# Leonhard111/M3L

Measured on AMD Instinct MI355X. Metric: MAE fwd+bwd samples/sec (image+tactile), higher is better.
Workload: dtype bf16; 1 GPU; BASELINE configs[1]: VTT vision+tactile MAE, 64x64 RGB + 2x32x32 tactile, ViT-Tiny 192/12/3/768 + decoder 192/4/3/768, mask 0.75; batch_per_gpu=256, global_batch=256, parallelism=dp1, grad_allreduce=none (one rank), rccl_ranks=0, step=zero_grad + mask + fwd + bwd + grad all-reduce + Adam

## Files before the change

### __graft_entry__.py

```python
import os
import subprocess
import sys

ROOT = os.path.dirname(os.path.abspath(__file__))
CSRC = os.path.join(ROOT, "m3l_amd", "csrc")
LIB = os.path.join(ROOT, "m3l_amd", "lib", "libm3l_amd.so")
SOURCES = ["gemm.hip", "wgrad.hip", "gemm_rowln.hip", "attention.hip", "attn_block.hip", "mlp_block.hip", "enc_mega.hip", "t192.hip", "conv.hip", "elementwise.hip", "mae_plan.hip", "mae_step.hip", "prof.hip", "err.hip", "comm.hip"]


OBJ = os.path.join(ROOT, "build", "obj")
HIPCC_FLAGS = ["--offload-arch=gfx950", "-O3", "-std=c++17", "-fPIC", "-Wno-unused-value", "-fno-slp-vectorize"]


def _headers():
    return [os.path.join(CSRC, f) for f in os.listdir(CSRC) if f.endswith((".h", ".cuh"))] + [os.path.join(ROOT, "include", "m3l_amd.h")]


def _compile_stale(force: bool):
    os.makedirs(OBJ, exist_ok=True)
    flags_file = os.path.join(OBJ, "flags.txt")
    flags = " ".join(HIPCC_FLAGS)
    if not os.path.exists(flags_file) or open(flags_file).read() != flags:
        force = True
        open(flags_file, "w").write(flags)
    hdr_t = max(os.path.getmtime(h) for h in _headers())
    jobs = []
    for src in SOURCES:
        obj = os.path.join(OBJ, src.replace(".hip", ".o"))
        s = os.path.join(CSRC, src)
        if force or not os.path.exists(obj) or os.path.getmtime(obj) < max(os.path.getmtime(s), hdr_t):
            jobs.append((src, ["hipcc"] + HIPCC_FLAGS + ["-c", s, "-o", obj]))
    running, failed = [], []
    while jobs or running:
        while jobs and len(running) < 8:
            src, cmd = jobs.pop(0)
            running.append((src, subprocess.Popen(cmd, cwd=CSRC, stdout=subprocess.PIPE, stderr=subprocess.STDOUT, text=True)))
        src, pr = running.pop(0)
        out, _ = pr.communicate()
        if pr.returncode != 0:
            failed.append(src)
# ... 88 lines not shown
```

### include/m3l_amd.h

```cpp
#ifndef M3L_AMD_H
#define M3L_AMD_H
#include <stddef.h>
#include <stdint.h>

#ifdef __cplusplus
extern "C" {
#endif

#define M3L_MAX_TACTILES 8

typedef struct m3l_geom {
    int image_h, image_w, image_patch, image_channels;
    int tactile_h, tactile_w, tactile_patch, tactile_channels;
    int num_tactiles;
    int use_vision;
    int use_tactile;
} m3l_geom;

typedef struct m3l_tf_cfg {
    int dim, depth, heads, mlp_dim;
    int project_out;
    int dtype;
    int dim_head;
} m3l_tf_cfg;

typedef struct m3l_dropout {
    float p;
    uint64_t seed;
} m3l_dropout;

int m3l_version(void);
int m3l_last_error(char* buf, size_t n);
int m3l_set_rowln(int enable);
int m3l_set_attn_block(int mode);
int m3l_set_enc_mega(int mode);
void m3l_set_attn_phase_buffer(void* dev_buf);
int m3l_set_defer_join(int on);
int m3l_set_wgrad_inline(int on);
int m3l_side_join(void* stream);
int m3l_comm_available(void);
int m3l_comm_unique_id(void* out128);
int m3l_comm_init(const void* id128, int rank, int world);
int m3l_comm_world(void);
int m3l_comm_allreduce(float* buf, size_t count, void* after_stream);
int m3l_comm_destroy(void);
int m3l_side_fork(void* after_stream, void** side_out);
int m3l_side_mark_pending(void);
void* m3l_side_stream(void);
int m3l_side_pending(void);
int m3l_set_drop_h(int on);
int m3l_set_t192(int on);
int m3l_set_t192_tt(int tt);
int m3l_set_residual_bf16(int on);
int m3l_set_t192_stagger(int lead_mask, int prio_mask);

int m3l_mask_counts(const m3l_geom* g, double ratio, int* counts_host);
int m3l_mask_sample(const m3l_geom* g, double ratio, int B, const float* const* noise, int64_t* masked, int64_t* unmasked,
                    void* stream);

int m3l_mask_sample_counts(const m3l_geom* g, int nm_img, int nm_tac, int B, const float* const* noise, int64_t* masked,
                           int64_t* unmasked, void* stream);

size_t m3l_embed_ws_bytes(const m3l_geom* g, int D, int dtype, int B, int L);
int m3l_embed_fwd(const m3l_geom* g, int D, int dtype, int B, int L, int cnt_img, const int64_t* idx, const float* image,
                  const float* const* tactiles, const void* const* tensors, void* ws, float* tokens, void* stream);
int m3l_embed_bwd(const m3l_geom* g, int D, int dtype, int B, int L, int cnt_img, const int64_t* idx, const float* image,
                  const float* const* tactiles, const void* const* tensors, void* ws, const float* dtokens, float* const* grads,
                  void* stream);

size_t m3l_transformer_ws_bytes(const m3l_tf_cfg* c, int B, int n);
int m3l_transformer_fwd(const m3l_tf_cfg* c, int B, int n, const float* x_in, const void* const* tensors, void* ws, void* y_t,
// ... 155 lines not shown
```

### m3l_amd/_lib.py

```python
import ctypes as C
import os

_HERE = os.path.dirname(os.path.abspath(__file__))
LIB_PATH = os.environ.get("M3L_LIB_PATH") or os.path.join(_HERE, "lib", "libm3l_amd.so")

c_p = C.c_void_p
c_i = C.c_int
c_sz = C.c_size_t


class Geom(C.Structure):
    _fields_ = [(n, c_i) for n in ("image_h", "image_w", "image_patch", "image_channels", "tactile_h", "tactile_w",
                                   "tactile_patch", "tactile_channels", "num_tactiles", "use_vision", "use_tactile")]


class CnnCfg(C.Structure):
    _fields_ = [(n, c_i) for n in ("in_channels", "height", "width", "dim", "tactile", "dtype")]


class TfCfg(C.Structure):
    _fields_ = [(n, c_i) for n in ("dim", "depth", "heads", "mlp_dim", "project_out", "dtype", "dim_head")]


class MaeCfg(C.Structure):
    _fields_ = [("geom", Geom), ("enc", TfCfg), ("dec", TfCfg), ("masking_ratio", C.c_double), ("early_conv", c_i), ("learned_pos", c_i)]


class Dropout(C.Structure):
    _fields_ = [("p", C.c_float), ("seed", C.c_uint64)]


class CommPlan(C.Structure):
    _fields_ = [("flat", c_p), ("total", C.c_long), ("min_bucket", C.c_long), ("layers_per_chunk", c_i), ("n_stages", c_i),
                ("stage_end", C.POINTER(C.c_long)), ("sent_out", C.POINTER(C.c_long))]


_SIGS = {
    "m3l_version": (c_i, []),
    "m3l_last_error": (c_i, [C.c_char_p, c_sz]),
    "m3l_set_rowln": (c_i, [c_i]),
    "m3l_set_attn_block": (c_i, [c_i]),
    "m3l_set_attn_phase_buffer": (None, [c_p]),
    "m3l_set_enc_mega": (c_i, [c_i]),
    "m3l_set_drop_h": (c_i, [c_i]),
    "m3l_set_direct_conv": (c_i, [c_i]),
    "m3l_set_t192": (c_i, [c_i]),
    "m3l_set_t192_tt": (c_i, [c_i]),
    "m3l_set_t192_stagger": (c_i, [c_i, c_i]),
    "m3l_set_residual_bf16": (c_i, [c_i]),
    "m3l_set_defer_join": (c_i, [c_i]),
    "m3l_set_wgrad_inline": (c_i, [c_i]),
    "m3l_side_join": (c_i, [c_p]),
    "m3l_side_stream": (c_p, []),
    "m3l_side_fork": (c_i, [c_p, C.POINTER(c_p)]),
    "m3l_side_mark_pending": (c_i, []),
    "m3l_comm_available": (c_i, []),
    "m3l_comm_unique_id": (c_i, [c_p]),
    "m3l_comm_init": (c_i, [c_p, c_i, c_i]),
    "m3l_comm_world": (c_i, []),
    "m3l_comm_allreduce": (c_i, [c_p, c_sz, c_p]),
    "m3l_comm_destroy": (c_i, []),
    "m3l_side_pending": (c_i, []),
    "m3l_mask_counts": (c_i, [C.POINTER(Geom), C.c_double, C.POINTER(c_i)]),
    "m3l_mask_sample": (c_i, [C.POINTER(Geom), C.c_double, c_i, c_p, c_p, c_p, c_p]),
    "m3l_mask_sample_counts": (c_i, [C.POINTER(Geom), c_i, c_i, c_i, c_p, c_p, c_p, c_p]),
    "m3l_embed_ws_bytes": (c_sz, [C.POINTER(Geom), c_i, c_i, c_i, c_i]),
    "m3l_embed_fwd": (c_i, [C.POINTER(Geom), c_i, c_i, c_i, c_i, c_i, c_p, c_p, c_p, c_p, c_p, c_p, c_p]),
    "m3l_embed_bwd": (c_i, [C.POINTER(Geom), c_i, c_i, c_i, c_i, c_i, c_p, c_p, c_p, c_p, c_p, c_p, c_p, c_p]),
    "m3l_transformer_ws_bytes": (c_sz, [C.POINTER(TfCfg), c_i, c_i]),
    "m3l_transformer_fwd": (c_i, [C.POINTER(TfCfg), c_i, c_i, c_p, c_p, c_p, c_p, c_p, c_p]),
    "m3l_transformer_bwd": (c_i, [C.POINTER(TfCfg), c_i, c_i, c_p, c_p, c_p, c_p, c_i, c_p, c_p, c_p]),
    "m3l_transformer_bwd_range": (c_i, [C.POINTER(TfCfg), c_i, c_i, c_p, c_p, c_p, c_p, c_i, c_p, c_p, c_i, c_i, c_p]),
    "m3l_transformer_ws_bytes_dropout": (c_sz, [C.POINTER(TfCfg), c_i, c_i, C.POINTER(Dropout)]),
    "m3l_transformer_fwd_dropout": (c_i, [C.POINTER(TfCfg), c_i, c_i, c_p, c_p, c_p, c_p, c_p, C.POINTER(Dropout), c_p]),
    "m3l_transformer_bwd_dropout": (c_i, [C.POINTER(TfCfg), c_i, c_i, c_p, c_p, c_p, c_p, c_i, c_p, c_p, C.POINTER(Dropout), c_p]),
    "m3l_transformer_bwd_range_dropout": (c_i, [C.POINTER(TfCfg), c_i, c_i, c_p, c_p, c_p, c_p, c_i, c_p, c_p, c_i, c_i, C.POINTER(Dropout), c_p]),
    "m3l_frozen_vit_ws_bytes": (c_sz, [C.POINTER(TfCfg), c_i, c_i]),
    "m3l_frozen_vit_fwd": (c_i, [C.POINTER(TfCfg), C.c_float, c_i, c_i, c_p, c_p, c_p, c_p, c_p]),
    "m3l_unshuffle_ws_bytes": (c_sz, [C.POINTER(Geom), c_i, c_i, c_i, c_i, c_i, c_i]),
    "m3l_unshuffle_fwd": (c_i, [C.POINTER(Geom), c_i, c_i, c_i, c_i, c_i, c_i, c_p, c_p, c_p, c_p, c_p, c_p, c_p, c_p]),
    "m3l_unshuffle_bwd": (c_i, [C.POINTER(Geom), c_i, c_i, c_i, c_i, c_i, c_i, c_p, c_p, c_p, c_p, c_p, c_p, c_p,
                                C.POINTER(c_i), c_p, c_p]),
    "m3l_heads_ws_bytes": (c_sz, [C.POINTER(Geom), c_i, c_i, c_i, c_i]),
    "m3l_heads_loss_fwd": (c_i, [C.POINTER(Geom), c_i, c_i, c_i, c_i, c_i, c_i, c_p, c_p, c_p, c_p, c_p, c_p, c_p, c_p, c_p,
# ... 106 lines not shown
```

### m3l_amd/csrc/elementwise.hip

```cpp
#include "common.cuh"
#include "kernels.h"
#include <cstring>
#include <vector>

namespace {

constexpr int MAXV = 16;
constexpr int WPB = 4;

__device__ __forceinline__ void store_val(float* p, float v) { *p = v; }
__device__ __forceinline__ void store_val(bf16* p, float v) { *p = (bf16)v; }


template <typename TO> __device__ __forceinline__ void store4(TO* p, f32x4 v);
template <> __device__ __forceinline__ void store4<float>(float* p, f32x4 v) { *reinterpret_cast<f32x4*>(p) = v; }
template <> __device__ __forceinline__ void store4<bf16>(bf16* p, f32x4 v) {
    bf16x4 o;
    o[0] = (bf16)v[0]; o[1] = (bf16)v[1]; o[2] = (bf16)v[2]; o[3] = (bf16)v[3];
    *reinterpret_cast<bf16x4*>(p) = o;
}
__device__ __forceinline__ f32x4 load4(const float* p) { return *reinterpret_cast<const f32x4*>(p); }
__device__ __forceinline__ f32x4 load4(const bf16* p) {
    const bf16x4 v = *reinterpret_cast<const bf16x4*>(p);
    return f32x4{(float)v[0], (float)v[1], (float)v[2], (float)v[3]};
}

template <int MAXC, typename TX>
__device__ __forceinline__ void row_stats(const TX* xr, int D, int lane, f32x4 (&v)[MAXC], float eps, float& mean, float& rstd) {
    float s = 0.f;
#pragma unroll
    for (int i = 0; i < MAXC; ++i) {
        const int e = 4 * (lane + 64 * i);
        v[i] = load4(xr + min(e, D - 4));
        if (e >= D) v[i] = f32x4{0.f, 0.f, 0.f, 0.f};
// ... 537 lines not shown
__global__ void vt_tactile_kernel(const TI* __restrict__ in, int B, int th, int tw, int S, int fs, float lo, float span, VtTactileOut o) {
    const long i = (long)blockIdx.x * blockDim.x + threadIdx.x;
    const int CH = 3 * S * fs;
    if (i >= (long)B * CH * th * tw) return;
    const int px = (int)(i % ((long)th * tw)), ch = (int)((i / ((long)th * tw)) % CH), b = (int)(i / ((long)th * tw * CH));
    const int f = ch / (3 * S), r = ch % (3 * S), s = r / 3, c = r % 3;
    o.p[s][(((long)b * 3 * fs) + f * 3 + c) * th * tw + px] = __fdiv_rn((float)in[i] - lo, span);
}

__global__ void mask_rank_kernel(MaskRankArgs a, int64_t* __restrict__ masked, int masked_ld, int64_t* __restrict__ unmasked,
                                 int unmasked_ld) {
    extern __shared__ float keys[];
    const int b = blockIdx.x;
    const MaskRankGroup gr = a.g[blockIdx.y];
    const float* __restrict__ noise = gr.noise;
    const int n = gr.n, nm = gr.nm, token_offset = gr.token_offset, masked_off = gr.masked_off, unmasked_off = gr.unmasked_off;
    for (int i = threadIdx.x; i < n; i += blockDim.x) keys[i] = noise[(long)b * n + i];
    __syncthreads();
    for (int i = threadIdx.x; i < n; i += blockDim.x) {
        const float k = keys[i];
        int rank = 0;
        for (int j = 0; j < n; ++j) {
            const float o = keys[j];
            rank += (o < k) || (o == k && j < i);
        }
        const int64_t tok = (int64_t)(i + token_offset);
        if (rank < nm)
            masked[(long)b * masked_ld + masked_off + rank] = tok;
        else
            unmasked[(long)b * unmasked_ld + unmasked_off + rank - nm] = tok;
    }
}

__device__ __forceinline__ void patch_locate(const PatchGroup& pg, const int64_t* idx, int idx_ld, int j0, int cnt, int row,
                                             int& b, int& s, int& ph, int& pw, int& local) {
    b = row / cnt;
    const int jj = row % cnt;
    const int tok = idx ? (int)idx[(long)b * idx_ld + j0 + jj] : pg.base + jj;
    local = tok - pg.base;
    s = local / pg.npatch;
    const int pidx = local % pg.npatch;
    const int gw = pg.W / pg.P;
    ph = pidx / gw;
    pw = pidx % gw;
}
__device__ __forceinline__ const float* patch_base(const PatchGroup& pg, int b, int s, int ph, int pw) {
    const float* src = pg.src[0];
#pragma unroll
    for (int i = 1; i < M3L_MAX_SENSORS; ++i) src = (s == i) ? pg.src[i] : src;
    return src + ((long)b * pg.C * pg.H + ph * pg.P) * pg.W + pw * pg.P;
}
struct PatchDiv {
    unsigned m_pp, m_p;
    int pp;
};
__device__ __forceinline__ PatchDiv patch_div(const PatchGroup& pg) {
    PatchDiv d;
    d.pp = pg.P * pg.P;
    d.m_pp = 0xFFFFFFFFu / (unsigned)d.pp + 1u;
    d.m_p = 0xFFFFFFFFu / (unsigned)pg.P + 1u;
    return d;
}
__device__ __forceinline__ int patch_off_t(const PatchGroup& pg, const PatchDiv& dv, int t, int& e) {
    const int c = (int)__umulhi((unsigned)t, dv.m_pp);
    const int rem = t - c * dv.pp;
    const int p1 = (int)__umulhi((unsigned)rem, dv.m_p);
    const int p2 = rem - p1 * pg.P;
    e = rem * pg.C + c;
    return (c * pg.H + p1) * pg.W + p2;
}
template <int NV>
__device__ __forceinline__ void patch_stage_stats(const PatchGroup& pg, const PatchDiv& dv, const float* __restrict__ base, int lane, int pd,
                                                  float eps, float* __restrict__ my, float& mean, float& rstd) {
    float v[NV];
    int ei[NV];
#pragma unroll
    for (int i = 0; i < NV; ++i) v[i] = base[patch_off_t(pg, dv, min(lane + 64 * i, pd - 1), ei[i])];
    float sum = 0.f;
#pragma unroll
    for (int i = 0; i < NV; ++i) {
        if (lane + 64 * i < pd) my[ei[i]] = v[i];
        else v[i] = 0.f;
        sum += v[i];
    }
    mean = wave_sum(sum) / pd;
    float q = 0.f;
#pragma unroll
    for (int i = 0; i < NV; ++i) {
        const float d = (lane + 64 * i < pd) ? v[i] - mean : 0.f;
        q += d * d;
    }
    rstd = rsqrtf(wave_sum(q) / pd + eps);
}

template <typename T, int NV>
__global__ __launch_bounds__(256) void patch_ln_kernel(PatchGroup pg, const int64_t* __restrict__ idx, int idx_ld, int j0, int cnt,
                                                         int rows, const float* __restrict__ gamma, const float* __restrict__ beta,
                                                         float eps, T* __restrict__ xn, int pdpad, int vec) {
    __shared__ __attribute__((aligned(16))) float buf[WPB][NV * 64];
    const int lane = threadIdx.x & 63, wave = threadIdx.x >> 6, row = blockIdx.x * WPB + wave;
    const int pd = pg.C * pg.P * pg.P;
    const PatchDiv dv = patch_div(pg);
    float* my = buf[wave];
// ... 1139 lines not shown
```

### m3l_amd/csrc/kernels.h

```cpp
#pragma once
#include <hip/hip_runtime.h>
#include <stddef.h>
#include <stdint.h>

#define M3L_MAX_SENSORS 8
#define M3L_MAX_PARTIAL_BLOCKS 2048


struct DropCtx {
    uint32_t thr;
    float scale;
    uint32_t k0, k1;
    uint32_t ctr2;
    int on;
};
DropCtx m3l_drop_ctx(float p, uint64_t seed, int layer, int site);

struct ProfScope {
    int idx;
    hipStream_t stream;
    ProfScope(const char* kind, long a, long b, long c, double work, hipStream_t st, double bytes = 0.0);
    ~ProfScope();
};

// ... 204 lines not shown
                  float gscale, hipStream_t st);
int m3l_adamw_flat(float* p, float* g, float* m, float* v, long n, float lr, float b1, float b2, float eps, float wd, int step, float gscale,
                   float max_norm, float* norm_ws, int scale_grads, hipStream_t st);
int m3l_adam_flat_dev(float* p, const float* g, float* m, float* v, long n, float lr, float b1, float b2, float eps, float wd,
                      int* step_dev, float* bc_dev, hipStream_t st);
struct MaskRankGroup { const float* noise; int n, nm, token_offset, masked_off, unmasked_off; };
struct MaskRankArgs { MaskRankGroup g[M3L_MAX_SENSORS + 1]; int count; };
int m3l_mask_rank_groups(const MaskRankArgs* args, int B, int64_t* masked, int masked_ld, int64_t* unmasked, int unmasked_ld, hipStream_t st);
int m3l_mask_rank(const float* noise, int B, int n, int nm, int token_offset, int64_t* masked, int masked_ld, int masked_off,
                  int64_t* unmasked, int unmasked_ld, int unmasked_off, hipStream_t st);
int m3l_patch_ln(int dtype, const PatchGroup* pg, const int64_t* idx, int idx_ld, int j0, int cnt, int B, const float* gamma,
                 const float* beta, float eps, void* xn, int pdpad, hipStream_t st);
int m3l_patch_ln_bwd(int dtype, const PatchGroup* pg, const int64_t* idx, int idx_ld, int j0, int cnt, int B, float eps,
                     const void* dxn, int pdpad, float* part_ws, float* dgamma, float* dbeta, int accumulate, hipStream_t st);
int m3l_embed_finalize(const float* E, int D, const PatchGroup* pg, const int64_t* idx, int idx_ld, int j0, int cnt, int B,
                       const float* gamma, const float* beta, float eps, const float* mod, int mod0, const float* pos, float* tokens,
                       int L, hipStream_t st);
int m3l_embed_finalize_bwd(int dtype, const float* dtok, int L, const float* E, int D, const PatchGroup* pg, const int64_t* idx,
                           int idx_ld, int j0, int cnt, int B, const float* gamma, float eps, void* dE, float* part_ws, float* dgamma,
                           float* dbeta, float* dmod, int mod0, int accumulate, hipStream_t st);
int k_unshuffle_fwd(const float* src, const float* mask_token, const int64_t* unmasked, int nvis, const int64_t* masked, int nmask,
                      int B, int dd, int n_img, int n_tac, const float* dmod, const float* pos_img, const float* pos_tac, float* dec_in,
                      hipStream_t st);
int k_unshuffle_bwd(const float* dY, const int64_t* unmasked, int nvis, const int64_t* masked, int nmask, int B, int dd, int n_img,
                      int n_tac, int nmod, float* dsrc, float* part_ws, float* dmask_token, float* ddmod, int accumulate, hipStream_t st);
int m3l_gather_rows(int dtype, const void* src, int N, int D, const int64_t* idx, int idx_ld, int j0, int cnt, int B, void* dst,
                    hipStream_t st);
int m3l_gather_rows2(int dtype, const void* src, int N, int D, const int64_t* idx, int idx_ld, int cnt0, int cnt1, int B, void* dst0, void* dst1,
                     hipStream_t st);
int m3l_scatter_rows2(int dtype, const void* src0, const void* src1, int N, int D, const int64_t* idx, int idx_ld, int cnt0, int cnt1, int B,
                      const float* scale_dev, void* dst, hipStream_t st);
int m3l_scatter_rows(int dtype, const void* src, int N, int D, const int64_t* idx, int idx_ld, int j0, int cnt, int B, void* dst,
                     hipStream_t st);
int m3l_mse(int dtype, const float* pred, int pdpad, const PatchGroup* pg, const int64_t* idx, int idx_ld, int j0, int cnt, int B,
            float weight, float* part_ws, int* nblocks_out, void* dpred, float* target_out, hipStream_t st);
```

### m3l_amd/csrc/mae_plan.hip

```cpp
#include <stdarg.h>
#include <stdio.h>
#include <stdlib.h>
#include <string.h>

#include <algorithm>
#include <map>
#include <mutex>
#include <vector>

#include "../../include/m3l_amd.h"
#include "common.cuh"
#include "kernels.h"


namespace {

constexpr float LN_EPS = 1e-5f;

struct SideStream {
    hipStream_t s = nullptr;
    std::vector<hipEvent_t> ev;
    int next = 0;
};
std::mutex g_side_mu;
// ... 10 lines not shown
    int prio_least = 0, prio_greatest = 0;
    M3L_HIP(hipDeviceGetStreamPriorityRange(&prio_least, &prio_greatest));
    M3L_HIP(hipStreamCreateWithPriority(&ss.s, hipStreamNonBlocking, prio_least));
    ss.ev.resize(64);
    for (auto& e : ss.ev) M3L_HIP(hipEventCreateWithFlags(&e, hipEventDisableTiming));
    return 0;
}
int g_defer_join = 0;
std::vector<hipEvent_t> g_pending;
std::map<const void*, std::vector<hipEvent_t>> g_set_done;
std::vector<hipEvent_t> g_tail_ring;
int g_tail_next = 0;
hipEvent_t tail_event() {
    std::lock_guard<std::mutex> lock(g_side_mu);
    if (g_tail_ring.empty()) {
        g_tail_ring.resize(16);
        for (auto& e : g_tail_ring) (void)hipEventCreateWithFlags(&e, hipEventDisableTiming);
    }
    hipEvent_t e = g_tail_ring[g_tail_next];
    g_tail_next = (g_tail_next + 1) % (int)g_tail_ring.size();
    return e;
}
hipEvent_t side_event() {
    std::lock_guard<std::mutex> lock(g_side_mu);
    hipEvent_t e = g_side.ev[g_side.next];
    g_side.next = (g_side.next + 1) % (int)g_side.ev.size();
    return e;
}

int g_wgrad_inline = -1;
bool wgrad_inline() {
    if (g_wgrad_inline < 0) g_wgrad_inline = getenv("M3L_WGRAD_INLINE") != nullptr && atoi(getenv("M3L_WGRAD_INLINE")) > 0 ? 1 : 0;
    return g_wgrad_inline > 0;
}
struct SideSection {
    bool on = false;
    int fork(hipStream_t st, hipStream_t* s) {
        *s = st;
        if (!g_defer_join || wgrad_inline()) return 0;
        if (side_init()) return 2;
        hipEvent_t ready = side_event();
        M3L_HIP(hipEventRecord(ready, st));
        M3L_HIP(hipStreamWaitEvent(g_side.s, ready, 0));
        *s = g_side.s;
        on = true;
        return 0;
    }
    int end() {
        if (!on) return 0;
        hipEvent_t tail = tail_event();
        M3L_HIP(hipEventRecord(tail, g_side.s));
        std::lock_guard<std::mutex> lock(g_side_mu);
        g_pending.push_back(tail);
        on = false;
        return 0;
    }
};

struct Arena {
    char* base;
    size_t off = 0;
    explicit Arena(void* b) : base(reinterpret_cast<char*>(b)) {}
    void* take(size_t bytes) {
        off = (off + 255) & ~size_t(255);
        void* p = base ? base + off : nullptr;
        off += bytes;
// ... 202 lines not shown
    for (int i = 0; i < w.nset; ++i) w.scratch2[i] = a.take_n<float>((size_t)std::max(std::max(m3l_gemm_nt_colsum_rows((int)M, (int)mlp), B), t192_rows_max) * mlp);
    w.ln_part_stride = (size_t)std::max(std::max(m3l_ln_bwd_blocks((int)M), B), t192_tiles_max) * 3 * D;
    w.ln_part = a.take_n<float>((size_t)(2 * c->depth + 1) * w.ln_part_stride);
    w.dpart = nullptr;
    if (dropout) {
        w.dp3.resize(w.nset);
        w.dp1.resize(w.nset);
        for (int i = 0; i < w.nset; ++i) {
            w.dp3[i] = a.take(M * D * e);
            w.dp1[i] = a.take(M * D * e);
        }
        w.dpart = a.take_n<float>((size_t)m3l_dropout_bwd_blocks((int)M) * D);
    }
    w.total = a.off + 256;
    return w;
}
int check_tf(const m3l_tf_cfg* c, int B, int n) {
    M3L_CHECK(c->dtype == 0 || c->dtype == 1, "transformer: bad dtype %d", c->dtype);
    M3L_CHECK(c->dim > 0 && c->dim % 8 == 0 && c->dim <= 1024, "transformer: dim=%d must be a multiple of 8, <= 1024", c->dim);
    M3L_CHECK(c->mlp_dim > 0 && c->mlp_dim % 8 == 0, "transformer: mlp_dim=%d must be a multiple of 8", c->mlp_dim);
    M3L_CHECK(c->heads > 0 && c->depth >= 0, "transformer: heads=%d depth=%d", c->heads, c->depth);
    M3L_CHECK(c->dim_head == 0 || c->dim_head == 32 || c->dim_head == 64 || c->dim_head == 128,
              "transformer: dim_head=%d is not one of 32, 64, 128 (0 = 64)", c->dim_head);
    M3L_CHECK(c->project_out || c->heads * tf_dh(c) == c->dim, "transformer: identity to_out needs heads*dim_head == dim");
    M3L_CHECK(c->dim % 64 == 0, "transformer: dim=%d must be a multiple of 64 (LDS-DMA GEMM K-tile)", c->dim);
    M3L_CHECK(B > 0 && n > 0, "transformer: empty input B=%d n=%d", B, n);
    return 0;
}

}

extern "C" {

int m3l_version(void) { return 402; }

int m3l_set_wgrad_inline(int on) {
    const int old = wgrad_inline() ? 1 : 0;
    g_wgrad_inline = on ? 1 : 0;
    return old;
}

void* m3l_side_stream(void) {
    if (side_init()) return nullptr;
    return (void*)g_side.s;
}

int m3l_side_fork(void* after_stream, void** side_out) {
    if (side_init()) return 2;
    hipEvent_t ready = side_event();
    M3L_HIP(hipEventRecord(ready, (hipStream_t)after_stream));
    M3L_HIP(hipStreamWaitEvent(g_side.s, ready, 0));
    *side_out = (void*)g_side.s;
    return 0;
}
int m3l_side_mark_pending(void) {
    if (side_init()) return 2;
    hipEvent_t tail = tail_event();
    M3L_HIP(hipEventRecord(tail, g_side.s));
    std::lock_guard<std::mutex> lock(g_side_mu);
    g_pending.push_back(tail);
    return 0;
}

int m3l_set_defer_join(int on) {
    const int old = g_defer_join;
    g_defer_join = on ? 1 : 0;
    return old;
// ... 817 lines not shown
    void *w, *wT, *dg, *dpred, *dpred_s, *ddg;
    float* pred;
};
struct HeadWs {
    HeadGroupWs g[2];
    float* loss_part;
    float* scratch;
    float* scratch_side;
    size_t scratch_b, total;
};
HeadWs head_layout(const Geo& ge, int dd, int dtype, int B, int nmask, void* ws) {
    Arena a(ws);
    HeadWs w;
    const size_t e = esz(dtype);
    const int pdp[2] = {ge.pdp_img, ge.pdp_tac};
    const size_t rows = (size_t)B * nmask;
    for (int i = 0; i < 2; ++i) {
        w.g[i].w = a.take((size_t)pdp[i] * dd * e);
        w.g[i].wT = a.take((size_t)dd * pdp[i] * e);
        w.g[i].dg = a.take(rows * dd * e);
        w.g[i].pred = a.take_n<float>(rows * pdp[i]);
        w.g[i].dpred = a.take(rows * pdp[i] * e);
        w.g[i].dpred_s = a.take(rows * pdp[i] * e);
        w.g[i].ddg = a.take(rows * dd * e);
    }
    w.loss_part = a.take_n<float>(2 * M3L_MAX_PARTIAL_BLOCKS);
    std::vector<std::pair<int, int>> shapes = {{ge.pdp_img, dd}, {ge.pdp_tac, dd}};
    w.scratch_b = scratch_bytes((int)std::max(rows, (size_t)1), shapes, std::max(dd, std::max(ge.pdp_img, ge.pdp_tac)));
    w.scratch = reinterpret_cast<float*>(a.take(w.scratch_b));
    w.scratch_side = reinterpret_cast<float*>(a.take(w.scratch_b));
    w.total = a.off + 256;
    return w;
}
}

size_t m3l_heads_ws_bytes(const m3l_geom* g, int dd, int dtype, int B, int nmask) {
    if (check_geom(g)) return 0;
    return head_layout(geo_of(g), dd, dtype, B, nmask, nullptr).total;
}

int m3l_heads_loss_fwd(const m3l_geom* g, int dd, int dtype, int B, int N, int nmask, int nm_img, const int64_t* masked,
                       const float* image, const float* const* tactiles, const void* dec_t, const void* const* tensors, void* ws,
                       float* loss, float* pred_img, float* tgt_img, float* pred_tac, float* tgt_tac, void* stream) {
    return m3l_heads_loss_fwd2(g, dd, dtype, B, N, nmask, nm_img, masked, image, tactiles, dec_t, tensors, ws, loss, nullptr, pred_img,
                               tgt_img, pred_tac, tgt_tac, stream);
}

int m3l_heads_loss_fwd2(const m3l_geom* g, int dd, int dtype, int B, int N, int nmask, int nm_img, const int64_t* masked,
                        const float* image, const float* const* tactiles, const void* dec_t, const void* const* tensors, void* ws,
                        float* loss, float* loss_parts, float* pred_img, float* tgt_img, float* pred_tac, float* tgt_tac, void* stream) {
    if (check_geom(g)) return 1;
    hipStream_t st = (hipStream_t)stream;
    const Geo ge = geo_of(g);
    HeadWs w = head_layout(ge, dd, dtype, B, nmask, ws);
    const int cnt[2] = {nm_img, nmask - nm_img}, j0[2] = {0, nm_img};
    const int pd[2] = {ge.pd_img, ge.pd_tac}, pdp[2] = {ge.pdp_img, ge.pdp_tac};
    const float weight[2] = {1.f, 10.f};
    const PatchGroup pgs[2] = {group_img(g, ge, image), group_tac(g, ge, tactiles)};
    float* tgt[2] = {tgt_img, tgt_tac};
    float* pred_out[2] = {pred_img, pred_tac};
    int nparts = 0;
    int part_beg[2] = {0, 0}, part_cnt[2] = {0, 0};
    {
        WeightPack pk;
        memset(&pk, 0, sizeof(pk));
        for (int i = 0; i < 2; ++i) {
            if (cnt[i] == 0) continue;
            pk.d[pk.count++] = WeightDesc{(const float*)tensors[2 * i], w.g[i].w, w.g[i].wT, pd[i], dd, dd, pdp[i]};
        }
        if (m3l_prep_weights(dtype, &pk, st)) return 1;
        if (m3l_prep_mode() == 1) return 0;
    }
    if (m3l_gather_rows2(dtype, dec_t, N, dd, masked, nmask, cnt[0], cnt[1], B, w.g[0].dg, w.g[1].dg, st)) return 1;
    for (int i = 0; i < 2; ++i) {
        if (cnt[i] == 0) continue;
        const int rows = B * cnt[i];
        GemmEpi e = epi0(pdp[i]);
        e.bias = (const float*)tensors[2 * i + 1];
        e.n_bias = pd[i];
        e.out_f32 = w.g[i].pred;
        if (m3l_gemm_nt(dtype, w.g[i].dg, dd, w.g[i].w, dd, rows, pdp[i], dd, &e, st)) return 1;
        int nb = 0;
        if (m3l_mse(dtype, w.g[i].pred, pdp[i], &pgs[i], masked, nmask, j0[i], cnt[i], B, weight[i], w.loss_part + nparts, &nb,
                    w.g[i].dpred, tgt[i], st))
            return 1;
        part_beg[i] = nparts; part_cnt[i] = nb;
        nparts += nb;
        if (pred_out[i])
            M3L_HIP(hipMemcpy2DAsync(pred_out[i], (size_t)pd[i] * 4, w.g[i].pred, (size_t)pdp[i] * 4, (size_t)pd[i] * 4, rows,
                                     hipMemcpyDeviceToDevice, st));
    }
    if (loss_parts) {
        M3L_HIP(hipMemsetAsync(loss_parts, 0, 2 * sizeof(float), st));
        for (int i = 0; i < 2; ++i)
            if (part_cnt[i] && m3l_reduce_rows(w.loss_part + part_beg[i], part_cnt[i], 1, 1, loss_parts + i, 0, st)) return 1;
    }
    return m3l_reduce_rows(w.loss_part, nparts, 1, 1, loss, 0, st);
}

int m3l_heads_loss_bwd(const m3l_geom* g, int dd, int dtype, int B, int N, int nmask, int nm_img, const int64_t* masked,
                       const void* const* tensors, void* ws, const float* dloss, void* d_dec, float* const* grads, void* stream) {
    if (check_geom(g)) return 1;
    (void)tensors;
    hipStream_t st = (hipStream_t)stream;
    const Geo ge = geo_of(g);
    HeadWs w = head_layout(ge, dd, dtype, B, nmask, ws);
    const int cnt[2] = {nm_img, nmask - nm_img}, j0[2] = {0, nm_img};
    const int pd[2] = {ge.pd_img, ge.pd_tac}, pdp[2] = {ge.pdp_img, ge.pdp_tac};
    M3L_HIP(hipMemsetAsync(d_dec, 0, (size_t)B * N * dd * esz(dtype), st));
    SideSection side;
    for (int i = 0; i < 2; ++i) {
        if (cnt[i] == 0) continue;
        const int rows = B * cnt[i];
        hipStream_t s2;
        if (side.fork(st, &s2)) return 2;
        const void* dpred = w.g[i].dpred;
        if (dloss) {
            if (m3l_scale_by_dev(dtype, w.g[i].dpred, (long)rows * pdp[i], dloss, w.g[i].dpred_s, s2)) return 1;
            dpred = w.g[i].dpred_s;
        }
        float* sc = side.on ? w.scratch_side : w.scratch;
        if (m3l_gemm_tn(dtype, dpred, pdp[i], w.g[i].dg, dd, rows, pdp[i], dd, sc, w.scratch_b, grads[2 * i], dd, pd[i], dd, 0, s2)) return 1;
        if (m3l_colsum(dtype, dpred, rows, pd[i], pdp[i], sc, grads[2 * i + 1], 0, s2)) return 1;
        GemmEpi e = epi0(dd);
        e.out_t = w.g[i].ddg;
        if (m3l_gemm_nt(dtype, w.g[i].dpred, pdp[i], w.g[i].wT, pdp[i], rows, dd, pdp[i], &e, st)) return 1;
    }
    if (m3l_scatter_rows2(dtype, w.g[0].ddg, w.g[1].ddg, N, dd, masked, nmask, cnt[0], cnt[1], B, dloss, d_dec, st)) return 1;
    return side.end();
}

namespace {
struct ConvL { int Ci, Co, KH, S, P, H, W, OH, OW, K, Kpad; long M; };
struct CnnWs {
    ConvL L[4];
    void *col[3], *act[3], *w[4], *wT[4];
    void *dout_t, *dpreA, *dpreB, *dcol;
    void *wf[3], *wd[3];
    float* slab;
    bool direct;
    float* scratch;
// ... 331 lines not shown
```

Before: 72620 samples/s.

## Fuse MAE pixel heads gather, GEMM and MSE loss into single kernels

Adds a fused forward kernel for the MAE output heads. It gathers masked decoder rows, runs the 192-wide head GEMM with MFMA, adds bias, computes the weighted MSE against the patchified targets and writes the bf16 dpred in one launch per step. A fused backward kernel computes d_dec from dpred times the transposed weights. It scatters the result directly to the masked tokens and zeroes the unmasked ones, replacing a full memset, per-group scale kernels and separate GEMMs. The path is on by default and limited to bf16 with dim 192. It adds redundant weight loads per block and a per-batch serial work loop in the backward kernel.

```diff
diff --git a/__graft_entry__.py b/__graft_entry__.py
--- a/__graft_entry__.py
+++ b/__graft_entry__.py
@@ -5,7 +5,7 @@
 ROOT = os.path.dirname(os.path.abspath(__file__))
 CSRC = os.path.join(ROOT, "m3l_amd", "csrc")
 LIB = os.path.join(ROOT, "m3l_amd", "lib", "libm3l_amd.so")
-SOURCES = ["gemm.hip", "wgrad.hip", "gemm_rowln.hip", "attention.hip", "attn_block.hip", "mlp_block.hip", "enc_mega.hip", "t192.hip", "conv.hip", "elementwise.hip", "mae_plan.hip", "mae_step.hip", "prof.hip", "err.hip", "comm.hip"]
+SOURCES = ["gemm.hip", "wgrad.hip", "gemm_rowln.hip", "attention.hip", "attn_block.hip", "mlp_block.hip", "enc_mega.hip", "t192.hip", "conv.hip", "elementwise.hip", "heads.hip", "mae_plan.hip", "mae_step.hip", "prof.hip", "err.hip", "comm.hip"]
 
 
 OBJ = os.path.join(ROOT, "build", "obj")
diff --git a/include/m3l_amd.h b/include/m3l_amd.h
--- a/include/m3l_amd.h
+++ b/include/m3l_amd.h
@@ -37,6 +37,7 @@
 void m3l_set_attn_phase_buffer(void* dev_buf);
 int m3l_set_defer_join(int on);
 int m3l_set_wgrad_inline(int on);
+int m3l_set_fused_heads(int on);
 int m3l_side_join(void* stream);
 int m3l_comm_available(void);
 int m3l_comm_unique_id(void* out128);
diff --git a/m3l_amd/_lib.py b/m3l_amd/_lib.py
--- a/m3l_amd/_lib.py
+++ b/m3l_amd/_lib.py
@@ -50,6 +50,7 @@
     "m3l_set_residual_bf16": (c_i, [c_i]),
     "m3l_set_defer_join": (c_i, [c_i]),
     "m3l_set_wgrad_inline": (c_i, [c_i]),
+    "m3l_set_fused_heads": (c_i, [c_i]),
     "m3l_side_join": (c_i, [c_p]),
     "m3l_side_stream": (c_p, []),
     "m3l_side_fork": (c_i, [c_p, C.POINTER(c_p)]),
diff --git a/m3l_amd/csrc/elementwise.hip b/m3l_amd/csrc/elementwise.hip
--- a/m3l_amd/csrc/elementwise.hip
+++ b/m3l_amd/csrc/elementwise.hip
@@ -1,5 +1,6 @@
 #include "common.cuh"
 #include "kernels.h"
+#include "patch.cuh"
 #include <cstring>
 #include <vector>
 
@@ -603,43 +604,6 @@
     }
 }
 
-__device__ __forceinline__ void patch_locate(const PatchGroup& pg, const int64_t* idx, int idx_ld, int j0, int cnt, int row,
-                                             int& b, int& s, int& ph, int& pw, int& local) {
-    b = row / cnt;
-    const int jj = row % cnt;
-    const int tok = idx ? (int)idx[(long)b * idx_ld + j0 + jj] : pg.base + jj;
-    local = tok - pg.base;
-    s = local / pg.npatch;
-    const int pidx = local % pg.npatch;
-    const int gw = pg.W / pg.P;
-    ph = pidx / gw;
-    pw = pidx % gw;
-}
-__device__ __forceinline__ const float* patch_base(const PatchGroup& pg, int b, int s, int ph, int pw) {
-    const float* src = pg.src[0];
-#pragma unroll
-    for (int i = 1; i < M3L_MAX_SENSORS; ++i) src = (s == i) ? pg.src[i] : src;
-    return src + ((long)b * pg.C * pg.H + ph * pg.P) * pg.W + pw * pg.P;
-}
-struct PatchDiv {
-    unsigned m_pp, m_p;
-    int pp;
-};
-__device__ __forceinline__ PatchDiv patch_div(const PatchGroup& pg) {
-    PatchDiv d;
-    d.pp = pg.P * pg.P;
-    d.m_pp = 0xFFFFFFFFu / (unsigned)d.pp + 1u;
-    d.m_p = 0xFFFFFFFFu / (unsigned)pg.P + 1u;
-    return d;
-}
-__device__ __forceinline__ int patch_off_t(const PatchGroup& pg, const PatchDiv& dv, int t, int& e) {
-    const int c = (int)__umulhi((unsigned)t, dv.m_pp);
-    const int rem = t - c * dv.pp;
-    const int p1 = (int)__umulhi((unsigned)rem, dv.m_p);
-    const int p2 = rem - p1 * pg.P;
-    e = rem * pg.C + c;
-    return (c * pg.H + p1) * pg.W + p2;
-}
 template <int NV>
 __device__ __forceinline__ void patch_stage_stats(const PatchGroup& pg, const PatchDiv& dv, const float* __restrict__ base, int lane, int pd,
                                                   float eps, float* __restrict__ my, float& mean, float& rstd) {
diff --git a/m3l_amd/csrc/heads.hip b/m3l_amd/csrc/heads.hip
--- /dev/null
+++ b/m3l_amd/csrc/heads.hip
@@ -0,0 +1,303 @@
+#include "common.cuh"
+#include "kernels.h"
+#include "patch.cuh"
+#include <algorithm>
+#include <cstring>
+
+namespace {
+
+constexpr int HDD = 192;
+constexpr int HT = 32;
+constexpr int RT = HT / 16;
+constexpr int WR = HT / 4;
+constexpr int A_LD = HDD + 8;
+constexpr int PPR = HDD / 8;
+
+struct HeadsFwdGroup {
+    const bf16* w;
+    const float* bias;
+    bf16* xn;
+    bf16* dpred;
+    float* pred_out;
+    float* tgt_out;
+    PatchGroup pg;
+    int j0, cnt, rows, pd, pdp, tiles;
+    float wt;
+};
+struct HeadsFwdArgs {
+    const bf16* dec;
+    const int64_t* idx;
+    int idx_ld, N;
+    HeadsFwdGroup g[2];
+    float* part;
+};
+
+__global__ __launch_bounds__(256) void heads_fwd_kernel(HeadsFwdArgs a) {
+    extern __shared__ __attribute__((aligned(16))) char smem[];
+    bf16* xa = reinterpret_cast<bf16*>(smem);
+    float* pr = reinterpret_cast<float*>(smem);
+    __shared__ float red[4];
+    const bool second = (int)blockIdx.x >= a.g[0].tiles;
+    const HeadsFwdGroup& G = second ? a.g[1] : a.g[0];
+    const int r0 = ((int)blockIdx.x - (second ? a.g[0].tiles : 0)) * HT;
+    const int tid = threadIdx.x, lane = tid & 63, wave = tid >> 6, g4 = lane >> 4, i16 = lane & 15;
+
+    const PatchDiv dv = patch_div(G.pg);
+    float tv[WR][4];
+#pragma unroll
+    for (int rr = 0; rr < WR; ++rr) {
+        const int row = min(r0 + wave * WR + rr, G.rows - 1);
+        int b, s, ph, pw, local;
+        patch_locate(G.pg, a.idx, a.idx_ld, G.j0, G.cnt, row, b, s, ph, pw, local);
+        const float* base = patch_base(G.pg, b, s, ph, pw);
+#pragma unroll
+        for (int u = 0; u < 4; ++u) {
+            int e;
+            tv[rr][u] = 64 * u < G.pd ? base[patch_off_t(G.pg, dv, min(lane + 64 * u, G.pd - 1), e)] : 0.f;
+        }
+    }
+    for (int p = tid; p < HT * PPR; p += 256) {
+        const int r = p / PPR, c = p - r * PPR, row = r0 + r;
+        uint4 v = make_uint4(0u, 0u, 0u, 0u);
+        if (row < G.rows) {
+            const int b = row / G.cnt, jj = row - b * G.cnt;
+            const long tok = a.idx[(long)b * a.idx_ld + G.j0 + jj];
+            v = reinterpret_cast<const uint4*>(a.dec + ((long)b * a.N + tok) * HDD)[c];
+            reinterpret_cast<uint4*>(G.xn + (long)row * HDD)[c] = v;
+        }
+        *reinterpret_cast<uint4*>(xa + r * A_LD + c * 8) = v;
+    }
+    __syncthreads();
+
+    const int ntw = G.pdp >> 6;
+    f32x4 acc[RT][4];
+#pragma unroll
+    for (int r = 0; r < RT; ++r)
+#pragma unroll
+        for (int c = 0; c < 4; ++c) acc[r][c] = f32x4{0.f, 0.f, 0.f, 0.f};
+#pragma unroll 2
+    for (int k0 = 0; k0 < HDD; k0 += 32) {
+        Frag<bf16> bw[4];
+#pragma unroll
+        for (int c = 0; c < 4; ++c)
+            if (c < ntw) bw[c] = load_kc(G.w + (long)((wave * ntw + c) * 16 + i16) * HDD + k0 + 8 * g4);
+#pragma unroll
+        for (int r = 0; r < RT; ++r) {
+            const Frag<bf16> af = load_kc(xa + (r * 16 + i16) * A_LD + k0 + 8 * g4);
+#pragma unroll
+            for (int c = 0; c < 4; ++c)
+                if (c < ntw) acc[r][c] = mma16(af, bw[c], acc[r][c]);
+        }
+    }
+    __syncthreads();
+    const int pld = G.pdp + 4;
+#pragma unroll
+    for (int c = 0; c < 4; ++c) {
+        if (c >= ntw) break;
+        const int col = (wave * ntw + c) * 16 + i16;
+        const float bias = col < G.pd ? G.bias[col] : 0.f;
+#pragma unroll
+        for (int r = 0; r < RT; ++r)
+#pragma unroll
+            for (int q = 0; q < 4; ++q) pr[(r * 16 + 4 * g4 + q) * pld + col] = acc[r][c][q] + bias;
+    }
+    __syncthreads();
+
+    float lsum = 0.f;
+#pragma unroll
+    for (int rr = 0; rr < WR; ++rr) {
+        const int r = wave * WR + rr, row = r0 + r;
+        if (row >= G.rows) break;
+        float* prow = pr + r * pld;
+#pragma unroll
+        for (int u = 0; u < 4; ++u) {
+            const int t = lane + 64 * u;
+            if (64 * u >= G.pd) break;
+            if (t < G.pd) {
+                int e;
+                (void)patch_off_t(G.pg, dv, t, e);
+                const float p = prow[e], d = p - tv[rr][u];
+                lsum += d * d;
+                if (G.pred_out) G.pred_out[(long)row * G.pd + e] = p;
+                if (G.tgt_out) G.tgt_out[(long)row * G.pd + e] = tv[rr][u];
+                prow[e] = d;
+            }
+        }
+    }
+    lsum = wave_sum(lsum);
+    if (lane == 0) red[wave] = lsum;
+    __syncthreads();
+    if (tid == 0) a.part[blockIdx.x] = G.wt * (red[0] + red[1] + red[2] + red[3]);
+
+    const float s2 = 2.f * G.wt;
+    const int ppr = G.pdp >> 3;
+    for (int p = tid; p < HT * ppr; p += 256) {
+        const int r = p / ppr, c8 = (p - r * ppr) * 8, row = r0 + r;
+        if (row >= G.rows) break;
+        const f32x4 lo = *reinterpret_cast<const f32x4*>(pr + r * pld + c8);
+        const f32x4 hi = *reinterpret_cast<const f32x4*>(pr + r * pld + c8 + 4);
+        bf16x8 o;
+#pragma unroll
+        for (int j = 0; j < 8; ++j) o[j] = (bf16)(c8 + j < G.pd ? (j < 4 ? lo[j] : hi[j - 4]) * s2 : 0.f);
+        *reinterpret_cast<bf16x8*>(G.dpred + (long)row * G.pdp + c8) = o;
+    }
+}
+
+struct HeadsBwdGroup {
+    const bf16* dpred;
+    bf16* dpred_s;
+    const bf16* wT;
+    int j0, cnt, pdp;
+};
+struct HeadsBwdArgs {
+    const int64_t* idx;
+    int idx_ld, N, nmask;
+    const float* dloss;
+    bf16* d_dec;
+    HeadsBwdGroup g[2];
+};
+constexpr int BWD_MAX_N = 1024;
+
+constexpr int BCW = 64;
+constexpr int BLD = BCW + 8;
+
+__global__ __launch_bounds__(256) void heads_bwd_kernel(HeadsBwdArgs a) {
+    __shared__ unsigned char masked[BWD_MAX_N];
+    __shared__ __attribute__((aligned(16))) bf16 stage[4][16 * BLD];
+    const int b = blockIdx.x, n0 = blockIdx.y * BCW, tid = threadIdx.x, lane = tid & 63, wave = tid >> 6, g4 = lane >> 4, i16 = lane & 15;
+    const int64_t* idx = a.idx + (long)b * a.idx_ld;
+    bf16* out = a.d_dec + (long)b * a.N * HDD + n0;
+    for (int t = tid; t < a.N; t += 256) masked[t] = 0;
+    __syncthreads();
+    for (int j = tid; j < a.nmask; j += 256) masked[idx[j]] = 1;
+    __syncthreads();
+    for (int p = tid; p < a.N * (BCW / 8); p += 256) {
+        const int t = p / (BCW / 8);
+        if (!masked[t]) reinterpret_cast<uint4*>(out + (long)t * HDD)[p - t * (BCW / 8)] = make_uint4(0u, 0u, 0u, 0u);
+    }
+    const float sc = a.dloss ? *a.dloss : 1.f;
+    const bool scale_out = a.dloss && blockIdx.y == 0;
+    const int t0 = (a.g[0].cnt + 15) >> 4, njobs = t0 + ((a.g[1].cnt + 15) >> 4);
+    bf16* st = stage[wave];
+    for (int job = wave; job < njobs; job += 4) {
+        const bool second = job >= t0;
+        const HeadsBwdGroup& G = second ? a.g[1] : a.g[0];
+        const int j_base = (job - (second ? t0 : 0)) * 16;
+        const int ja = j_base + i16;
+        const long arow = (long)b * G.cnt + min(ja, G.cnt - 1);
+        f32x4 acc[BCW / 16];
+#pragma unroll
+        for (int c = 0; c < BCW / 16; ++c) acc[c] = f32x4{0.f, 0.f, 0.f, 0.f};
+        for (int k0 = 0; k0 < G.pdp; k0 += 32) {
+            const Frag<bf16> af = load_kc(G.dpred + arow * G.pdp + k0 + 8 * g4);
+            Frag<bf16> bw[BCW / 16];
+#pragma unroll
+            for (int c = 0; c < BCW / 16; ++c) bw[c] = load_kc(G.wT + (long)(n0 + c * 16 + i16) * G.pdp + k0 + 8 * g4);
+            if (scale_out && ja < G.cnt) {
+                bf16x8 s;
+#pragma unroll
+                for (int j = 0; j < 8; ++j) s[j] = (bf16)((float)af.v[j] * sc);
+                *reinterpret_cast<bf16x8*>(G.dpred_s + arow * G.pdp + k0 + 8 * g4) = s;
+            }
+#pragma unroll
+            for (int c = 0; c < BCW / 16; ++c) acc[c] = mma16(af, bw[c], acc[c]);
+        }
+#pragma unroll
+        for (int c = 0; c < BCW / 16; ++c)
+#pragma unroll
+            for (int q = 0; q < 4; ++q) st[(4 * g4 + q) * BLD + c * 16 + i16] = (bf16)(acc[c][q] * sc);
+        __builtin_amdgcn_wave_barrier();
+        for (int p = lane; p < 16 * (BCW / 8); p += 64) {
+            const int r = p / (BCW / 8), c = p - r * (BCW / 8), j = j_base + r;
+            if (j >= G.cnt) break;
+            const long tok = idx[G.j0 + j];
+            reinterpret_cast<uint4*>(out + tok * HDD)[c] = *reinterpret_cast<const uint4*>(st + r * BLD + c * 8);
+        }
+        __builtin_amdgcn_wave_barrier();
+    }
+}
+
+int g_fwd_lds_set = 0;
+
+}
+
+bool m3l_heads_fused_supported(int dtype, int dd, int B, int N, int nmask, int cnt0, int cnt1, int pd0, int pdp0, int pd1, int pdp1) {
+    if (dtype != 1 || dd != HDD || N > BWD_MAX_N || nmask <= 0 || nmask >= N) return false;
+    const int cnt[2] = {cnt0, cnt1}, pd[2] = {pd0, pd1}, pdp[2] = {pdp0, pdp1};
+    long tiles = 0;
+    for (int i = 0; i < 2; ++i) {
+        if (cnt[i] == 0) continue;
+        if (pdp[i] % 64 != 0 || pdp[i] > 256 || pd[i] > pdp[i] || pd[i] <= 0) return false;
+        tiles += cdiv((long)B * cnt[i], HT);
+    }
+    return tiles <= 2 * M3L_MAX_PARTIAL_BLOCKS;
+}
+
+int m3l_heads_fused_fwd(const void* dec, int N, const int64_t* idx, int idx_ld, int B, const int* j0, const int* cnt, const PatchGroup* pgs,
+                        const int* pd, const int* pdp, const float* weight, const void* const* w, const float* const* bias, void* const* xn,
+                        void* const* dpred, float* const* pred_out, float* const* tgt_out, float* part, int* tiles_out, hipStream_t st) {
+    HeadsFwdArgs a;
+    memset(&a, 0, sizeof(a));
+    a.dec = (const bf16*)dec;
+    a.idx = idx;
+    a.idx_ld = idx_ld;
+    a.N = N;
+    a.part = part;
+    int lds = HT * A_LD * 2;
+    for (int i = 0; i < 2; ++i) {
+        HeadsFwdGroup& g = a.g[i];
+        g.rows = B * cnt[i];
+        g.tiles = cdiv(g.rows, HT);
+        tiles_out[i] = g.tiles;
+        if (!g.rows) continue;
+        M3L_CHECK(pgs[i].nsrc > 0 && pgs[i].nsrc <= M3L_MAX_SENSORS && pgs[i].P > 0, "heads_fused_fwd: bad patch group");
+        M3L_CHECK(pgs[i].C * pgs[i].P * pgs[i].P == pd[i], "heads_fused_fwd: patch dim %d != %d", pgs[i].C * pgs[i].P * pgs[i].P, pd[i]);
+        g.w = (const bf16*)w[i];
+        g.bias = bias[i];
+        g.xn = (bf16*)xn[i];
+        g.dpred = (bf16*)dpred[i];
+        g.pred_out = pred_out[i];
+        g.tgt_out = tgt_out[i];
+        g.pg = pgs[i];
+        g.j0 = j0[i];
+        g.cnt = cnt[i];
+        g.pd = pd[i];
+        g.pdp = pdp[i];
+        g.wt = weight[i] / ((float)g.rows * (float)pd[i]);
+        lds = std::max(lds, HT * (pdp[i] + 4) * 4);
+    }
+    const int grid = a.g[0].tiles + a.g[1].tiles;
+    if (!grid) return 0;
+    if (!g_fwd_lds_set) {
+        M3L_HIP(hipFuncSetAttribute((const void*)heads_fwd_kernel, hipFuncAttributeMaxDynamicSharedMemorySize, HT * (256 + 4) * 4));
+        g_fwd_lds_set = 1;
+    }
+    heads_fwd_kernel<<<grid, 256, lds, st>>>(a);
+    M3L_LAUNCH_CHECK();
+    return 0;
+}
+
+int m3l_heads_fused_bwd(int N, int nmask, const int64_t* idx, int idx_ld, int B, const int* j0, const int* cnt, const int* pdp,
+                        const void* const* dpred, void* const* dpred_s, const void* const* wT, const float* dloss, void* d_dec, hipStream_t st) {
+    if (!B) return 0;
+    HeadsBwdArgs a;
+    memset(&a, 0, sizeof(a));
+    a.idx = idx;
+    a.idx_ld = idx_ld;
+    a.N = N;
+    a.nmask = nmask;
+    a.dloss = dloss;
+    a.d_dec = (bf16*)d_dec;
+    for (int i = 0; i < 2; ++i) {
+        a.g[i].cnt = cnt[i];
+        if (!cnt[i]) continue;
+        a.g[i].dpred = (const bf16*)dpred[i];
+        a.g[i].dpred_s = (bf16*)dpred_s[i];
+        a.g[i].wT = (const bf16*)wT[i];
+        a.g[i].j0 = j0[i];
+        a.g[i].pdp = pdp[i];
+    }
+    heads_bwd_kernel<<<dim3(B, HDD / BCW), 256, 0, st>>>(a);
+    M3L_LAUNCH_CHECK();
+    return 0;
+}
diff --git a/m3l_amd/csrc/kernels.h b/m3l_amd/csrc/kernels.h
--- a/m3l_amd/csrc/kernels.h
+++ b/m3l_amd/csrc/kernels.h
@@ -260,5 +260,11 @@
                       const float* scale_dev, void* dst, hipStream_t st);
 int m3l_scatter_rows(int dtype, const void* src, int N, int D, const int64_t* idx, int idx_ld, int j0, int cnt, int B, void* dst,
                      hipStream_t st);
+bool m3l_heads_fused_supported(int dtype, int dd, int B, int N, int nmask, int cnt0, int cnt1, int pd0, int pdp0, int pd1, int pdp1);
+int m3l_heads_fused_fwd(const void* dec, int N, const int64_t* idx, int idx_ld, int B, const int* j0, const int* cnt, const PatchGroup* pgs,
+                        const int* pd, const int* pdp, const float* weight, const void* const* w, const float* const* bias, void* const* xn,
+                        void* const* dpred, float* const* pred_out, float* const* tgt_out, float* part, int* tiles_out, hipStream_t st);
+int m3l_heads_fused_bwd(int N, int nmask, const int64_t* idx, int idx_ld, int B, const int* j0, const int* cnt, const int* pdp,
+                        const void* const* dpred, void* const* dpred_s, const void* const* wT, const float* dloss, void* d_dec, hipStream_t st);
 int m3l_mse(int dtype, const float* pred, int pdpad, const PatchGroup* pg, const int64_t* idx, int idx_ld, int j0, int cnt, int B,
             float weight, float* part_ws, int* nblocks_out, void* dpred, float* target_out, hipStream_t st);
diff --git a/m3l_amd/csrc/mae_plan.hip b/m3l_amd/csrc/mae_plan.hip
--- a/m3l_amd/csrc/mae_plan.hip
+++ b/m3l_amd/csrc/mae_plan.hip
@@ -66,6 +66,11 @@
 bool wgrad_inline() {
     if (g_wgrad_inline < 0) g_wgrad_inline = getenv("M3L_WGRAD_INLINE") != nullptr && atoi(getenv("M3L_WGRAD_INLINE")) > 0 ? 1 : 0;
     return g_wgrad_inline > 0;
+}
+int g_fused_heads = -1;
+bool fused_heads_on() {
+    if (g_fused_heads < 0) g_fused_heads = getenv("M3L_FUSED_HEADS") != nullptr && atoi(getenv("M3L_FUSED_HEADS")) <= 0 ? 0 : 1;
+    return g_fused_heads > 0;
 }
 struct SideSection {
     bool on = false;
@@ -334,7 +339,13 @@
 
 extern "C" {
 
-int m3l_version(void) { return 402; }
+int m3l_version(void) { return 403; }
+
+int m3l_set_fused_heads(int on) {
+    const int old = fused_heads_on() ? 1 : 0;
+    g_fused_heads = on ? 1 : 0;
+    return old;
+}
 
 int m3l_set_wgrad_inline(int on) {
     const int old = wgrad_inline() ? 1 : 0;
@@ -1218,6 +1229,10 @@
     w.total = a.off + 256;
     return w;
 }
+bool heads_fused(const Geo& ge, int dd, int dtype, int B, int N, int nmask, int nm_img) {
+    return fused_heads_on() &&
+           m3l_heads_fused_supported(dtype, dd, B, N, nmask, nm_img, nmask - nm_img, ge.pd_img, ge.pdp_img, ge.pd_tac, ge.pdp_tac);
+}
 }
 
 size_t m3l_heads_ws_bytes(const m3l_geom* g, int dd, int dtype, int B, int nmask) {
@@ -1257,6 +1272,17 @@
         if (m3l_prep_weights(dtype, &pk, st)) return 1;
         if (m3l_prep_mode() == 1) return 0;
     }
+    if (heads_fused(ge, dd, dtype, B, N, nmask, nm_img)) {
+        const void* wc[2] = {w.g[0].w, w.g[1].w};
+        const float* bias[2] = {(const float*)tensors[1], (const float*)tensors[3]};
+        void* xn[2] = {w.g[0].dg, w.g[1].dg};
+        void* dpred[2] = {w.g[0].dpred, w.g[1].dpred};
+        if (m3l_heads_fused_fwd(dec_t, N, masked, nmask, B, j0, cnt, pgs, pd, pdp, weight, wc, bias, xn, dpred, pred_out, tgt, w.loss_part,
+                                part_cnt, st))
+            return 1;
+        part_beg[1] = part_cnt[0];
+        nparts = part_cnt[0] + part_cnt[1];
+    } else {
     if (m3l_gather_rows2(dtype, dec_t, N, dd, masked, nmask, cnt[0], cnt[1], B, w.g[0].dg, w.g[1].dg, st)) return 1;
     for (int i = 0; i < 2; ++i) {
         if (cnt[i] == 0) continue;
@@ -1276,6 +1302,7 @@
             M3L_HIP(hipMemcpy2DAsync(pred_out[i], (size_t)pd[i] * 4, w.g[i].pred, (size_t)pdp[i] * 4, (size_t)pd[i] * 4, rows,
                                      hipMemcpyDeviceToDevice, st));
     }
+    }
     if (loss_parts) {
         M3L_HIP(hipMemsetAsync(loss_parts, 0, 2 * sizeof(float), st));
         for (int i = 0; i < 2; ++i)
@@ -1293,6 +1320,24 @@
     HeadWs w = head_layout(ge, dd, dtype, B, nmask, ws);
     const int cnt[2] = {nm_img, nmask - nm_img}, j0[2] = {0, nm_img};
     const int pd[2] = {ge.pd_img, ge.pd_tac}, pdp[2] = {ge.pdp_img, ge.pdp_tac};
+    if (heads_fused(ge, dd, dtype, B, N, nmask, nm_img)) {
+        const void* dpred[2] = {w.g[0].dpred, w.g[1].dpred};
+        void* dpred_s[2] = {w.g[0].dpred_s, w.g[1].dpred_s};
+        const void* wT[2] = {w.g[0].wT, w.g[1].wT};
+        if (m3l_heads_fused_bwd(N, nmask, masked, nmask, B, j0, cnt, pdp, dpred, dpred_s, wT, dloss, d_dec, st)) return 1;
+        SideSection side;
+        hipStream_t s2;
+        if (side.fork(st, &s2)) return 2;
+        float* sc = side.on ? w.scratch_side : w.scratch;
+        for (int i = 0; i < 2; ++i) {
+            if (cnt[i] == 0) continue;
+            const int rows = B * cnt[i];
+            const void* dp = dloss ? w.g[i].dpred_s : w.g[i].dpred;
+            if (m3l_gemm_tn(dtype, dp, pdp[i], w.g[i].dg, dd, rows, pdp[i], dd, sc, w.scratch_b, grads[2 * i], dd, pd[i], dd, 0, s2)) return 1;
+            if (m3l_colsum(dtype, dp, rows, pd[i], pdp[i], sc, grads[2 * i + 1], 0, s2)) return 1;
+        }
+        return side.end();
+    }
     M3L_HIP(hipMemsetAsync(d_dec, 0, (size_t)B * N * dd * esz(dtype), st));
     SideSection side;
     for (int i = 0; i < 2; ++i) {
diff --git a/m3l_amd/csrc/patch.cuh b/m3l_amd/csrc/patch.cuh
--- /dev/null
+++ b/m3l_amd/csrc/patch.cuh
@@ -0,0 +1,41 @@
+#pragma once
+#include "common.cuh"
+#include "kernels.h"
+
+__device__ __forceinline__ void patch_locate(const PatchGroup& pg, const int64_t* idx, int idx_ld, int j0, int cnt, int row,
+                                             int& b, int& s, int& ph, int& pw, int& local) {
+    b = row / cnt;
+    const int jj = row % cnt;
+    const int tok = idx ? (int)idx[(long)b * idx_ld + j0 + jj] : pg.base + jj;
+    local = tok - pg.base;
+    s = local / pg.npatch;
+    const int pidx = local % pg.npatch;
+    const int gw = pg.W / pg.P;
+    ph = pidx / gw;
+    pw = pidx % gw;
+}
+__device__ __forceinline__ const float* patch_base(const PatchGroup& pg, int b, int s, int ph, int pw) {
+    const float* src = pg.src[0];
+#pragma unroll
+    for (int i = 1; i < M3L_MAX_SENSORS; ++i) src = (s == i) ? pg.src[i] : src;
+    return src + ((long)b * pg.C * pg.H + ph * pg.P) * pg.W + pw * pg.P;
+}
+struct PatchDiv {
+    unsigned m_pp, m_p;
+    int pp;
+};
+__device__ __forceinline__ PatchDiv patch_div(const PatchGroup& pg) {
+    PatchDiv d;
+    d.pp = pg.P * pg.P;
+    d.m_pp = 0xFFFFFFFFu / (unsigned)d.pp + 1u;
+    d.m_p = 0xFFFFFFFFu / (unsigned)pg.P + 1u;
+    return d;
+}
+__device__ __forceinline__ int patch_off_t(const PatchGroup& pg, const PatchDiv& dv, int t, int& e) {
+    const int c = (int)__umulhi((unsigned)t, dv.m_pp);
+    const int rem = t - c * dv.pp;
+    const int p1 = (int)__umulhi((unsigned)rem, dv.m_p);
+    const int p2 = rem - p1 * pg.P;
+    e = rem * pg.C + c;
+    return (c * pg.H + p1) * pg.W + p2;
+}
```

New measurement: 73260 samples/s, median of 6. Within noise of the previous version (+0.9%).
